# CaiLiLab/MuRaL

Hardware: AMD Instinct MI355X
Metric: predicted bases/s (SNV local=10/distal=1000, 4-class, predict) (higher is better)
Workload: dtype f32; 1 GPU; SNV default predict, synthetic 10M positions (BASELINE.json configs[1]); local_radius=10, distal_radius=1000, n_class=4, input=2-bit packed genome resident in HBM, every site's full window, weights=weights_init, torch.manual_seed(0), parallelism=dp1, collective=none

## Files before the change

### mural_amd/csrc/snv.h

```cpp
#pragma once
#include "common.h"

namespace mural {

constexpr int SNV_C = 32;
constexpr int SNV_K = 3;
constexpr int SNV_NLAYER = 10;
constexpr int SNV_KSTEPS = 24;
constexpr int SNV_WFRAG = 2 * SNV_KSTEPS * 64;
constexpr int SNV_LUT = 125 * SNV_C;
constexpr int SNV_TAPS = 3 * N_SYM * SNV_C;
constexpr int SNV_LUTBLK = SNV_LUT + SNV_TAPS + SNV_C;
constexpr int SNV_LUT4 = 256 * SNV_C;
constexpr int SNV_MAXCLASS = 16;
constexpr int SNV_CHUNK = 131072;
constexpr int SNV_NB2MAX = 9;
constexpr int SNV_THREADS = 256;
constexpr int SNV_WAVES = SNV_THREADS / 64;
constexpr int SNV_MID_HALF = 100;

enum { L_RB1A_C1 = 0, L_RB1A_C2, L_RB1B_C1, L_RB1B_C2, L_CONV2, L_RB2A_C1, L_RB2A_C2, L_RB2B_C1, L_RB2B_C2, L_CONV3 };
enum { EX_RB1_ENTRY = 0, EX_BN_MID = 1, EX_BN_OUT = 2, EX_FC_BN = 3, EX_COUNT = 4 };

struct TowerGeom {
  int L1;
  int col0;
  int L[3];
  int pk[3], ps[3], pp[3];
  int Sc[3];
  int NC[3];
  int nb[3];
  FastDiv dL[3];
  FastDiv dSc[3];
};

struct TowerDev {
  const float* lut;
  const float* lut4;
  const float* taps;
  const float* bias0;
  const float* wfrag;
  const float* wfrag4;
  const float* bias;
  const float* post_s;
  const float* post_t;
  const float* ex_s;
  const float* ex_t;
  const float* fc_w;
  const float* fc_b;
};

struct LocalDev {
  const float* emb;
  const float* w1t;
  const float* b1;
  const float* w2t;
  const float* b2;
  const float* w3t;
  const float* b3;
  const float* frag;
  int frag_floats;
  int cols, emb_rows, in1, h1, h2, n_class;
};

struct LocalMfmaDims { int K1p, K2p, K3p, n1b, n2b, s1, sx, dbg; };

struct Stage1Tower { int L1, col0, L2, pk, ps, pp; };

struct Stage1Args {
  Stage1Tower tw[2];
  const float* lut[2];
  const float* lut4;
  int Lwin, cw, wave_bytes, x0_cols, nwords, radius;
  int64_t n;
  const uint8_t* codes;
  MuralGenome genome;
  const int64_t* pos;
  const uint8_t* strand;
  float* x0;
  const float* dense;
  int32_t* status;
  int loc_on;
  LocalDev loc;
  LocalMfmaDims loc_d;
  const int64_t* loc_cat;
  float* loc_out;
  int* zero;
  int site_mode;
  int dbg_alias;
};

constexpr int FIRST_TRAIN_MAXGRID = 256;
struct FirstFold {
  const float* dz;
  const float* x;
  const float* add1;
  const float* add2;
  const float* state;
  const float* gamma;
  const double* acc;
  double n;
  float* dgamma;
  float* dbeta;
};
struct FirstTrainArgs {
  Stage1Tower tw;
  int Lwin, cw, wave_bytes;
  int64_t B;
  const uint8_t* sym;
  const float* lutblk;
  float* y;
  uint8_t* arg;
  const float* dy;
  float* dpart;
  int cl;
  double* stat;
  FirstFold fold;
  int dbg;
  unsigned long long* stamps;
};
extern unsigned long long* g_first_stamps;
int first_train_grid(int64_t B);
bool first_train_supported(int C, int pk);
int launch_first_train(FirstTrainArgs a, bool bwd, hipStream_t stream);

struct SnvFwdArgs {
  TowerGeom geom[2];
  TowerDev tw[2];
  int P;
  int nbuf;
  int Lwin;
  int n_class;
  int has_local;
  int64_t n;
  const float* x0;
  int x0_cols;
  const float* local_logits;
  float* out;
  float* taps;
  int tap_stride;
  unsigned long long* stamps;
  const int32_t* status;
  int tw_first, tw_last;
  float* xlogit;
  int par;
  float* xlogit2;
  int* tile_count;
  int phase;
  float* s3[2];
  int wave;
  int* unit_counter;
  int seg_n, seg_step, seg_col0;
};

constexpr int RU_EC = 9;
constexpr int RU_EV = 5;
constexpr int RU_L = 2 * RU_EC;
constexpr int RU_SC = RU_L + 1;

struct EdgeArgs {
  TowerDev tw;
  int64_t n;
  const int64_t* pos;
  const uint8_t* strand;
  int64_t glen;
  int64_t t0[2], nb;
  int woff;
  int L1;
  int L2, L3;
  int D;
  int pk2, ps2, pp2;
  int u_lo, u_hi;
  int right_pad;
  const float* F[2];
  const float* El[2];
  const float* Er[2];
  const float* R[2];
  const float* S[2];
  float* s3;
};

constexpr int EW_P = 7;
size_t edge_wave_lds_bytes();
int launch_snv_edge_wave(const EdgeArgs& e, int* unit_counter, hipStream_t stream);

}

struct MuralSnvModel {
  MuralSnvShape shape;
  mural::SnvFwdArgs args;
  mural::SnvFwdArgs args_split[4];
  size_t lds_split[4];
  bool split;
  mural::SnvFwdArgs args_small;
  size_t lds_small;
  mural::LocalDev local;
  float* blob;
  size_t blob_floats;
  size_t lds_bytes;
  mural::Stage1Args s1;
  size_t s1_lds_bytes;
  bool s1_pair;
  bool loc_fused;
  mural::LocalMfmaDims loc_d;
  size_t loc_lds;
  bool longwin;
  bool front_only;
  bool front_mid;
  int lw_nA, lw_LA, lw_LB, lw_SB, lw_nj;
  mural::SnvFwdArgs args_lwA, args_lwB;
  size_t lds_lwA, lds_lwB;
  int64_t chunk;
};

namespace mural {
bool stage1_small_batch(int64_t n);
int launch_snv_stage1(const Stage1Args& a, bool packed, size_t lds_bytes, hipStream_t stream);
int launch_snv_local(const LocalDev& L, const int64_t* cat, int64_t n, float* out, hipStream_t stream);
int launch_snv_towers(const MuralSnvModel* m, const SnvFwdArgs& a, size_t lds_bytes, hipStream_t stream);
int profile_begin();
int profile_end(double* total_ms, int64_t* launches);
size_t plan_wave_geometry(SnvFwdArgs& a, int Lwin, int Pw, int n_class, int tower, int phase);
int launch_snv_tower_wave(const SnvFwdArgs& a, size_t lds_bytes, hipStream_t stream);
int launch_snv_tower_wave_jobs(const SnvFwdArgs* jobs, const size_t* lds_bytes, int n, hipStream_t stream);
extern unsigned long long* g_tower_stamps;
}
```

### mural_amd/csrc/snv_stage1.hip

```cpp
#include <algorithm>
#include <cstdlib>

#include "dense_symbol.h"
#include "snv.h"
#include "snv_local_mfma.h"

namespace mural {

using f32x4 = __attribute__((ext_vector_type(4))) float;
__device__ __forceinline__ f32x4 s1_ld4(const float* p) { return *reinterpret_cast<const f32x4*>(p); }
__device__ __forceinline__ f32x4 s1_max4(f32x4 a, f32x4 b) {
  return f32x4{fmaxf(a.x, b.x), fmaxf(a.y, b.y), fmaxf(a.z, b.z), fmaxf(a.w, b.w)};
}

constexpr int S1_WAVES = 16;
constexpr int S1_THREADS = 64 * S1_WAVES;

__device__ __forceinline__ void wave_lds_fence() { asm volatile("s_waitcnt lgkmcnt(0)" ::: "memory"); }

__device__ __forceinline__ uint32_t kmer_index(const uint8_t* cb, int j, int L1) {
  if (j <= 0 || j >= L1 - 1) return 255u;
  const uint32_t l = cb[j], c = cb[j + 1], r = cb[j + 2];
  return (l <= 4u && c <= 4u && r <= 4u) ? (25u * l + 5u * c + r) : 255u;
}

template <int SLOT>
__device__ __forceinline__ void build_kwin(const Stage1Tower& g, int lane, const uint8_t* cb0, uint8_t* kw, int nl = 64) {
  const uint8_t* cb = cb0 + g.col0;
  const int ndw = g.L2 * (SLOT / 4);
  for (int t = lane; t < ndw; t += nl) {
    const int j2 = t / (SLOT / 4);
    const int w0 = 4 * (t % (SLOT / 4));
    uint32_t packed = 0;
#pragma unroll
    for (int q = 0; q < 4; ++q) {
      const int w = w0 + q;
      const uint32_t idx = (w < g.pk) ? kmer_index(cb, j2 * g.ps - g.pp + w, g.L1) : 255u;
      packed |= idx << (8 * q);
    }
    *reinterpret_cast<uint32_t*>(kw + (size_t)t * 4) = packed;
  }
}

template <int SLOT>
__device__ __forceinline__ void pooled_lookup(const Stage1Tower& g, int lane, const float* lutS, const uint8_t* cb0,
                                              const uint8_t* kw, float* __restrict__ out , int nl = 64) {
  const float* tapS = lutS + SNV_LUT;
  const float* b0S = tapS + SNV_TAPS;
  const uint8_t* cb = cb0 + g.col0;
  const int cg = lane & 7;
  const int total = g.L2 * 8;
  for (int task = lane; task < total; task += nl) {
    const int jt = task >> 3;
    const int j2 = jt == 0 ? g.L2 - 1 : jt - 1;
    uint32_t d[SLOT / 4];
    if (SLOT == 16) {
      const uint4 q = *reinterpret_cast<const uint4*>(kw + (size_t)j2 * 16);
      d[0] = q.x; d[1] = q.y; d[2] = q.z; d[SLOT / 4 - 1] = q.w;
    } else {
      d[0] = *reinterpret_cast<const uint32_t*>(kw + (size_t)j2 * 4);
    }
    uint32_t hi = d[SLOT / 4 - 1] & 0x00FFFFFFu;
#pragma unroll
    for (int r = 0; r + 1 < SLOT / 4; ++r) hi |= d[r];
    const bool fast = ((hi & 0x80808080u) == 0u) && (g.pk == SLOT - 1);
    f32x4 m = f32x4{-INFINITY, -INFINITY, -INFINITY, -INFINITY};
    if (fast) {
#pragma unroll
      for (int w = 0; w < SLOT - 1; ++w) {
        const uint32_t idx = (d[w >> 2] >> (8 * (w & 3))) & 0xFFu;
        m = s1_max4(m, s1_ld4(lutS + idx * 32u + 4u * cg));
      }
    } else {
      const int jlo = j2 * g.ps - g.pp;
      for (int w = 0; w < g.pk; ++w) {
        const int j = jlo + w;
        if (j < 0 || j >= g.L1) continue;
        const uint32_t idx = kmer_index(cb, j, g.L1);
        f32x4 v;
        if (idx != 255u) {
          v = s1_ld4(lutS + idx * 32u + 4u * cg);
        } else {
          const uint32_t sl = (j == 0) ? (uint32_t)SYM_PAD : cb[j];
          const uint32_t sc = cb[j + 1];
          const uint32_t sr = (j == g.L1 - 1) ? (uint32_t)SYM_PAD : cb[j + 2];
          v = s1_ld4(b0S + 4 * cg);
          v += s1_ld4(tapS + (0 * N_SYM + sl) * 32 + 4 * cg);
          v += s1_ld4(tapS + (1 * N_SYM + sc) * 32 + 4 * cg);
          v += s1_ld4(tapS + (2 * N_SYM + sr) * 32 + 4 * cg);
        }
        m = s1_max4(m, v);
      }
    }
    *reinterpret_cast<f32x4*>(out + (size_t)j2 * 32 + 4 * cg) = m;
  }
}

__device__ __forceinline__ void build_kpair(const Stage1Tower& g, int lane, const uint8_t* cb0, uint8_t* kw) {
  const uint8_t* cb = cb0 + g.col0;
  for (int t = lane; t < 2 * g.L2; t += 64) {
    const int j2 = t >> 1, half = t & 1;
    const int j0 = j2 * g.ps - g.pp + 8 * half;
    const int ncol = half ? 7 : 8;
    uint32_t sy[10];
    uint32_t bad = (j0 < 1 || j0 + ncol - 1 > g.L1 - 2) ? 1u : 0u;
#pragma unroll
    for (int i = 0; i < 10; ++i) {
      const int idx = j0 + i;
      const bool in = idx >= 0 && idx <= g.L1 + 1 && i < ncol + 2;
      sy[i] = in ? cb[idx] : 0u;
      if (i < ncol + 2 && (!in || sy[i] > 3u)) bad = 1u;
    }
    uint32_t lo = 0;
#pragma unroll
    for (int q = 0; q < 4; ++q) {
      uint32_t code;
      if (half && q == 3) code = 25u * sy[6] + 5u * sy[7] + sy[8];
      else code = 64u * sy[2 * q] + 16u * sy[2 * q + 1] + 4u * sy[2 * q + 2] + sy[2 * q + 3];
      lo |= (code & 0xFFu) << (8 * q);
    }
    uint32_t* dst = reinterpret_cast<uint32_t*>(kw + (size_t)j2 * 16 + 8 * half);
    dst[0] = lo;
    dst[1] = bad;
  }
}

__device__ __forceinline__ void pooled_lookup_pair(const Stage1Tower& g, int lane, const float* lutS, const float* lut4S, const uint8_t* cb0,
                                                   const uint8_t* kw, float* __restrict__ out ) {
  const float* tapS = lutS + SNV_LUT;
  const float* b0S = tapS + SNV_TAPS;
  const uint8_t* cb = cb0 + g.col0;
  const int cg = lane & 7;
  const int total = g.L2 * 8;
  for (int task = lane; task < total; task += 64) {
    const int jt = task >> 3;
    const int j2 = jt == 0 ? g.L2 - 1 : jt - 1;
    const uint4 q = *reinterpret_cast<const uint4*>(kw + (size_t)j2 * 16);
    f32x4 m;
    if (((q.y | q.w) & 0xFFu) == 0u) {
      m = s1_ld4(lut4S + (q.x & 0xFFu) * 32u + 4u * cg);
      m = s1_max4(m, s1_ld4(lut4S + ((q.x >> 8) & 0xFFu) * 32u + 4u * cg));
      m = s1_max4(m, s1_ld4(lut4S + ((q.x >> 16) & 0xFFu) * 32u + 4u * cg));
      m = s1_max4(m, s1_ld4(lut4S + (q.x >> 24) * 32u + 4u * cg));
      m = s1_max4(m, s1_ld4(lut4S + (q.z & 0xFFu) * 32u + 4u * cg));
      m = s1_max4(m, s1_ld4(lut4S + ((q.z >> 8) & 0xFFu) * 32u + 4u * cg));
      m = s1_max4(m, s1_ld4(lut4S + ((q.z >> 16) & 0xFFu) * 32u + 4u * cg));
      m = s1_max4(m, s1_ld4(lutS + (q.z >> 24) * 32u + 4u * cg));
    } else {
      m = f32x4{-INFINITY, -INFINITY, -INFINITY, -INFINITY};
      const int jlo = j2 * g.ps - g.pp;
      for (int w = 0; w < g.pk; ++w) {
        const int j = jlo + w;
        if (j < 0 || j >= g.L1) continue;
        const uint32_t idx = kmer_index(cb, j, g.L1);
        f32x4 v;
        if (idx != 255u) {
          v = s1_ld4(lutS + idx * 32u + 4u * cg);
        } else {
          const uint32_t sl = (j == 0) ? (uint32_t)SYM_PAD : cb[j];
          const uint32_t sc = cb[j + 1];
          const uint32_t sr = (j == g.L1 - 1) ? (uint32_t)SYM_PAD : cb[j + 2];
          v = s1_ld4(b0S + 4 * cg);
          v += s1_ld4(tapS + (0 * N_SYM + sl) * 32 + 4 * cg);
          v += s1_ld4(tapS + (1 * N_SYM + sc) * 32 + 4 * cg);
          v += s1_ld4(tapS + (2 * N_SYM + sr) * 32 + 4 * cg);
        }
        m = s1_max4(m, v);
      }
    }
    *reinterpret_cast<f32x4*>(out + (size_t)j2 * 32 + 4 * cg) = m;
  }
}

template <int SRC>
__global__ __launch_bounds__(S1_THREADS) void snv_stage1_kernel(const Stage1Args args) {
  extern __shared__ __attribute__((aligned(16))) float s1mem[];
  const int tid = threadIdx.x;
  const int lane = tid & 63;
  const int wave = __builtin_amdgcn_readfirstlane(tid >> 6);
  float* lutL = s1mem;
  float* lutM = s1mem + SNV_LUTBLK;
  const bool pair = args.lut4 != nullptr;
  float* lut4 = s1mem + 2 * SNV_LUTBLK;
  uint8_t* wbase = reinterpret_cast<uint8_t*>(s1mem + 2 * SNV_LUTBLK + (pair ? SNV_LUT4 : 0)) + (size_t)wave * args.wave_bytes;
  uint8_t* cb = wbase;
  uint8_t* kwL = cb + args.cw;
  uint8_t* kwM = kwL + args.tw[0].L2 * 16;

  for (int i = tid * 4; i < SNV_LUTBLK; i += S1_THREADS * 4) {
    *reinterpret_cast<f32x4*>(lutL + i) = s1_ld4(args.lut[0] + i);
    *reinterpret_cast<f32x4*>(lutM + i) = s1_ld4(args.lut[1] + i);
  }
  if (pair)
    for (int i = tid * 4; i < SNV_LUT4; i += S1_THREADS * 4) *reinterpret_cast<f32x4*>(lut4 + i) = s1_ld4(args.lut4 + i);
  __syncthreads();

  const int Lwin = args.Lwin;
  const int64_t stride = (int64_t)gridDim.x * S1_WAVES;
  int64_t row = (int64_t)blockIdx.x * S1_WAVES + wave;
  int64_t pos_pre = 0;
  uint32_t neg_pre = 0;
  if (SRC == 1 && row < args.n) {
    pos_pre = args.pos[row];
    neg_pre = args.strand[row];
  }
  for (; row < args.n; row += stride) {
    if (SRC == 1) {
      const int64_t ws = pos_pre - args.radius;
      const bool neg = neg_pre != 0;
      const int64_t glen = args.genome.length;
      if (row + stride < args.n) {
        pos_pre = args.pos[row + stride];
        neg_pre = args.strand[row + stride];
      }
      if (lane == 0) {
        cb[0] = SYM_PAD;
        cb[Lwin + 1] = SYM_PAD;
      }
      for (int wi = lane; wi < args.nwords; wi += 64) {
        const int64_t w = (ws >> 4) + wi;
        uint32_t word = 0, mword = 0;
        if (w >= 0 && 16 * w < glen) {
          word = args.genome.packed2[w];
          mword = (args.genome.nmask[w >> 1] >> (16u * (uint32_t)(w & 1))) & 0xFFFFu;
        }
        const int j0 = (int)(16 * w - ws);
        if (w < 0 || 16 * w >= glen) mword = 0xFFFFu;
        else if (16 * w + 15 >= glen) mword |= 0xFFFFu << (uint32_t)(glen - 16 * w);
        const uint32_t cw = neg ? ~word : word;
        const int jb = neg ? Lwin - 1 - j0 - 15 : j0;
        uint8_t* dst = cb + jb + 1;
        const bool nfree = (mword & 0xFFFFu) == 0u;
#pragma unroll
        for (int k = 0; k < 16; ++k) {
          const int o = neg ? 15 - k : k;
          uint32_t sym = (cw >> (2 * k)) & 3u;
          if (!nfree) sym = ((mword >> k) & 1u) ? (uint32_t)SYM_N : sym;
          if ((unsigned)(jb + o) < (unsigned)Lwin) dst[o] = (uint8_t)sym;
        }
      }
      if (args.genome.n_amb > 0) {
        const int64_t e0 = amb_lower_bound_wave(args.genome.amb_pos, args.genome.n_amb, ws, lane);
        for (int64_t e = e0 + lane; e < args.genome.n_amb; e += 64) {
          const int64_t gpos = args.genome.amb_pos[e];
          if (gpos >= ws + Lwin) break;
          uint32_t sym = args.genome.amb_sym[e];
          if (neg) sym = sym_complement(sym);
          cb[(int)(neg ? (ws + Lwin - 1 - gpos) : (gpos - ws)) + 1] = (uint8_t)sym;
        }
      }
    } else {
      const uint8_t* src = args.codes + row * Lwin;
      for (int jj = lane; jj < Lwin + 2; jj += 64) {
        const int j = jj - 1;
        cb[jj] = (j >= 0 && j < Lwin) ? src[j] : (uint8_t)SYM_PAD;
      }
    }
    wave_lds_fence();
    if (pair) build_kpair(args.tw[0], lane, cb, kwL);
    else build_kwin<16>(args.tw[0], lane, cb, kwL);
    build_kwin<4>(args.tw[1], lane, cb, kwM);
    wave_lds_fence();
    float* out = args.x0 + (size_t)(args.dbg_alias ? (row & 63) : row) * args.x0_cols * 32;
    if (pair) pooled_lookup_pair(args.tw[0], lane, lutL, lut4, cb, kwL, out);
    else pooled_lookup<16>(args.tw[0], lane, lutL, cb, kwL, out);
    pooled_lookup<4>(args.tw[1], lane, lutM, cb, kwM, out + (size_t)args.tw[0].L2 * 32);
    wave_lds_fence();
  }
}

template <int SRC>
__global__ __launch_bounds__(S1_THREADS) void snv_stage1_site_kernel(const Stage1Args args) {
  extern __shared__ __attribute__((aligned(16))) float s1mem[];
  const int tid = threadIdx.x;
  if (args.loc_on && (int64_t)blockIdx.x == args.n) {
    if (tid < LOC_THREADS) local_mlp_mfma_body(args.loc, args.loc_cat, args.n, args.loc_out, args.loc_d, s1mem, 0, 1);
    return;
  }
  float* lutL = s1mem;
  float* lutM = s1mem + SNV_LUTBLK;
  uint8_t* cb = reinterpret_cast<uint8_t*>(s1mem + 2 * SNV_LUTBLK);
  uint8_t* kwL = cb + args.cw;
  uint8_t* kwM = kwL + args.tw[0].L2 * 16;
  for (int i = tid * 4; i < SNV_LUTBLK; i += S1_THREADS * 4) {
    *reinterpret_cast<f32x4*>(lutL + i) = s1_ld4(args.lut[0] + i);
    *reinterpret_cast<f32x4*>(lutM + i) = s1_ld4(args.lut[1] + i);
  }
  const int Lwin = args.Lwin;
  if (args.zero != nullptr && blockIdx.x == 0)
    for (int64_t i = tid; i < args.n; i += S1_THREADS) args.zero[i] = 0;
  for (int64_t row = blockIdx.x; row < args.n; row += gridDim.x) {
    __syncthreads();
    if (SRC == 1) {
      const int64_t ws = args.pos[row] - args.radius;
      const bool neg = args.strand[row] != 0;
      if (tid == 0) {
        cb[0] = SYM_PAD;
        cb[Lwin + 1] = SYM_PAD;
      }
      for (int j = tid; j < Lwin; j += S1_THREADS) {
        const int64_t gpos = neg ? ws + Lwin - 1 - j : ws + j;
        uint32_t sym = genome_sym_iupac(args.genome, gpos);
        if (neg) sym = sym_complement(sym);
        cb[j + 1] = (uint8_t)sym;
      }
    } else if (SRC == 2) {
      const float* src = args.dense + (size_t)row * 4 * Lwin;
      if (tid == 0) {
        cb[0] = SYM_PAD;
        cb[Lwin + 1] = SYM_PAD;
      }
      bool bad = false;
      for (int j0 = tid; j0 < Lwin; j0 += 2 * S1_THREADS) {
        const int j1 = j0 + S1_THREADS;
        const int j1c = j1 < Lwin ? j1 : j0;
        float v[2][4];
#pragma unroll
        for (int ch = 0; ch < 4; ++ch) {
          v[0][ch] = src[(size_t)ch * Lwin + j0];
          v[1][ch] = src[(size_t)ch * Lwin + j1c];
        }
        int s0 = dense_symbol(v[0][0], v[0][1], v[0][2], v[0][3]);
        int s1 = dense_symbol(v[1][0], v[1][1], v[1][2], v[1][3]);
        bad |= (s0 < 0) | (s1 < 0);
        cb[j0 + 1] = (uint8_t)(s0 < 0 ? SYM_N : s0);
        if (j1 < Lwin) cb[j1 + 1] = (uint8_t)(s1 < 0 ? SYM_N : s1);
      }
      if (bad && args.status != nullptr) atomicOr(args.status, (int)MURAL_E_ENCODING);
    } else {
      const uint8_t* src = args.codes + row * Lwin;
      for (int jj = tid; jj < Lwin + 2; jj += S1_THREADS) {
        const int j = jj - 1;
        cb[jj] = (j >= 0 && j < Lwin) ? src[j] : (uint8_t)SYM_PAD;
      }
    }
    __syncthreads();
    build_kwin<16>(args.tw[0], tid, cb, kwL, S1_THREADS);
    build_kwin<4>(args.tw[1], tid, cb, kwM, S1_THREADS);
    __syncthreads();
    float* out = args.x0 + (size_t)row * args.x0_cols * 32;
    pooled_lookup<16>(args.tw[0], tid, lutL, cb, kwL, out, S1_THREADS);
    pooled_lookup<4>(args.tw[1], tid, lutM, cb, kwM, out + (size_t)args.tw[0].L2 * 32, S1_THREADS);
  }
}


template <int SLOT>
__device__ __forceinline__ void pooled_lookup_train(const Stage1Tower& g, int lane, const float* lutS, const uint8_t* cb0,
                                                    const uint8_t* kw, float* __restrict__ y ,
                                                    uint8_t* __restrict__ arg , int cl, f32x4& sum1, f32x4& sum2) {
  const float* tapS = lutS + SNV_LUT;
  const float* b0S = tapS + SNV_TAPS;
  const uint8_t* cb = cb0 + g.col0;
  const int cg = lane & 7;
  const int total = g.L2 * 8;
  for (int task = lane; task < total; task += 64) {
    const int j2 = task >> 3;
    uint32_t d[SLOT / 4];
    if (SLOT == 16) {
      const uint4 q = *reinterpret_cast<const uint4*>(kw + (size_t)j2 * 16);
      d[0] = q.x; d[1] = q.y; d[2] = q.z; d[SLOT / 4 - 1] = q.w;
    } else {
      d[0] = *reinterpret_cast<const uint32_t*>(kw + (size_t)j2 * 4);
    }
    uint32_t hi = d[SLOT / 4 - 1] & 0x00FFFFFFu;
#pragma unroll
    for (int r = 0; r + 1 < SLOT / 4; ++r) hi |= d[r];
    const bool fast = ((hi & 0x80808080u) == 0u) && (g.pk == SLOT - 1);
    float m[4] = {-INFINITY, -INFINITY, -INFINITY, -INFINITY};
    uint32_t am[4] = {0u, 0u, 0u, 0u};
    if (fast) {
#pragma unroll
      for (int w = 0; w < SLOT - 1; ++w) {
        const uint32_t idx = (d[w >> 2] >> (8 * (w & 3))) & 0xFFu;
        const f32x4 v = s1_ld4(lutS + idx * 32u + 4u * cg);
#pragma unroll
        for (int q = 0; q < 4; ++q) {
          const bool gt = v[q] > m[q];
          m[q] = gt ? v[q] : m[q];
          am[q] = gt ? (uint32_t)w : am[q];
        }
      }
    } else {
      const int jlo = j2 * g.ps - g.pp;
      for (int w = 0; w < g.pk; ++w) {
        const int j = jlo + w;
        if (j < 0 || j >= g.L1) continue;
        const uint32_t idx = kmer_index(cb, j, g.L1);
        f32x4 v;
        if (idx != 255u) {
          v = s1_ld4(lutS + idx * 32u + 4u * cg);
        } else {
          const uint32_t sl = (j == 0) ? (uint32_t)SYM_PAD : cb[j];
          const uint32_t sc = cb[j + 1];
          const uint32_t sr = (j == g.L1 - 1) ? (uint32_t)SYM_PAD : cb[j + 2];
          v = s1_ld4(b0S + 4 * cg);
          v += s1_ld4(tapS + (0 * N_SYM + sl) * 32 + 4 * cg);
          v += s1_ld4(tapS + (1 * N_SYM + sc) * 32 + 4 * cg);
          v += s1_ld4(tapS + (2 * N_SYM + sr) * 32 + 4 * cg);
        }
#pragma unroll
        for (int q = 0; q < 4; ++q) {
          const bool gt = v[q] > m[q];
          m[q] = gt ? v[q] : m[q];
          am[q] = gt ? (uint32_t)w : am[q];
        }
      }
    }
    if (cl) {
      *reinterpret_cast<f32x4*>(y + (size_t)j2 * 32 + 4 * cg) = f32x4{m[0], m[1], m[2], m[3]};
      const f32x4 r = f32x4{fmaxf(m[0], 0.f), fmaxf(m[1], 0.f), fmaxf(m[2], 0.f), fmaxf(m[3], 0.f)};
      sum1 += r;
      sum2 += f32x4{r.x * r.x, r.y * r.y, r.z * r.z, r.w * r.w};
    } else {
#pragma unroll
      for (int q = 0; q < 4; ++q) y[(size_t)(4 * cg + q) * g.L2 + j2] = m[q];
    }
    *reinterpret_cast<uint32_t*>(arg + (size_t)j2 * 32 + 4 * cg) = am[0] | (am[1] << 8) | (am[2] << 16) | (am[3] << 24);
  }
}

template <int SLOT>
__device__ __forceinline__ void pooled_scatter(const Stage1Tower& g, int lane, float* acc, const uint8_t* cb0,
                                               const uint8_t* kw, const float* __restrict__ dy ,
                                               const uint8_t* __restrict__ arg , int cl) {
  float* tapA = acc + SNV_LUT;
  float* b0A = tapA + SNV_TAPS;
  const uint8_t* cb = cb0 + g.col0;
  const int cg = lane & 7;
  const int total = g.L2 * 8;
  float bsum[4] = {0.f, 0.f, 0.f, 0.f};
  constexpr int NT = 6;
  for (int t0 = lane; t0 < total; t0 += 64 * NT) {
    uint32_t awv[NT];
    f32x4 gv[NT];
#pragma unroll
    for (int u = 0; u < NT; ++u) {
      const int task = t0 + 64 * u;
      const int j2 = (task < total ? task : t0) >> 3;
      awv[u] = *reinterpret_cast<const uint32_t*>(arg + (size_t)j2 * 32 + 4 * cg);
      if (cl) {
        gv[u] = *reinterpret_cast<const f32x4*>(dy + (size_t)j2 * 32 + 4 * cg);
      } else {
#pragma unroll
        for (int q = 0; q < 4; ++q) gv[u][q] = dy[(size_t)(4 * cg + q) * g.L2 + j2];
      }
    }
#pragma unroll
    for (int u = 0; u < NT; ++u) {
      const int task = t0 + 64 * u;
      if (task >= total) break;
      const int j2 = task >> 3;
      const uint32_t aw = awv[u];
      const int jlo = j2 * g.ps - g.pp;
#pragma unroll
      for (int q = 0; q < 4; ++q) {
        const int c = 4 * cg + q;
        const float gq = gv[u][q];
        const int w = (int)((aw >> (8 * q)) & 0xFFu);
        const uint32_t idx = kw[(size_t)j2 * SLOT + w];
        bsum[q] += gq;
        if (idx != 255u) {
          atomicAdd(&acc[idx * 32u + c], gq);
        } else {
          const int j = jlo + w;
          const uint32_t sl = (j == 0) ? (uint32_t)SYM_PAD : cb[j];
          const uint32_t sc = cb[j + 1];
          const uint32_t sr = (j == g.L1 - 1) ? (uint32_t)SYM_PAD : cb[j + 2];
          atomicAdd(&tapA[(0 * N_SYM + sl) * 32 + c], gq);
          atomicAdd(&tapA[(1 * N_SYM + sc) * 32 + c], gq);
          atomicAdd(&tapA[(2 * N_SYM + sr) * 32 + c], gq);
        }
      }
    }
  }
#pragma unroll
  for (int q = 0; q < 4; ++q) {
    float v = bsum[q];
    v += __shfl_xor(v, 8);
    v += __shfl_xor(v, 16);
    v += __shfl_xor(v, 32);
    if (lane < 8) atomicAdd(&b0A[4 * cg + q], v);
  }
}

#define FT_STAMP(K) do { if (a.stamps && tid == 0) a.stamps[8 * blockIdx.x + (K)] = __builtin_amdgcn_s_memrealtime(); } while (0)


template <int SLOT>
__device__ __forceinline__ void pooled_scatter_cl(const Stage1Tower& g, int lane, float* acc, const uint8_t* cb0, const uint8_t* kw,
                                                  const float* __restrict__ dy , const uint8_t* __restrict__ arg ,
                                                  int dbg) {
  float* tapA = acc + SNV_LUT;
  float* b0A = tapA + SNV_TAPS;
  const uint8_t* cb = cb0 + g.col0;
  const int c = lane & 31, h = lane >> 5;
  const int npair = (g.L2 + 1) >> 1;
  float bsum = 0.f;
  const __amdgpu_buffer_rsrc_t gd = __builtin_amdgcn_make_buffer_rsrc(const_cast<float*>(dy), 0, (dbg & 2) ? 0 : g.L2 * 128, 0x00020000);
  const __amdgpu_buffer_rsrc_t ad = __builtin_amdgcn_make_buffer_rsrc(const_cast<uint8_t*>(arg), 0, (dbg & 2) ? 0 : g.L2 * 32, 0x00020000);
  constexpr int NT = 16;
  for (int p0 = 0; p0 < npair; p0 += NT) {
    float gv[NT];
    uint32_t awv[NT];
    const uint32_t go = 4u * (uint32_t)lane + 256u * (uint32_t)p0, ao = (uint32_t)lane + 64u * (uint32_t)p0;
    int hh = h;
    asm volatile("" : "+v"(hh));
#pragma unroll
    for (int u = 0; u < NT; ++u) {
      awv[u] = __builtin_amdgcn_raw_buffer_load_b8(ad, ao + 64u * u, 0, 0);
      gv[u] = __builtin_bit_cast(float, __builtin_amdgcn_raw_buffer_load_b32(gd, go + 256u * u, 0, 0));
    }
#pragma unroll
    for (int u = 0; u < NT; ++u) {
      const int j2 = 2 * (p0 + u) + hh;
      if (j2 < g.L2) {
        const float gq = gv[u];
        const int w = (int)(awv[u] & 0xFFu);
        const uint32_t idx = (dbg & 4) ? (uint32_t)(j2 & 63) : kw[j2 * SLOT + w];
        bsum += gq;
        if (dbg & 1) continue;
        const int j = j2 * g.ps - g.pp + w;
        const uint32_t sl = (j == 0) ? (uint32_t)SYM_PAD : cb[j];
        const bool tab = idx != 255u;
        atomicAdd(tab ? &acc[idx * 32u + c] : &tapA[(0 * N_SYM + sl) * 32 + c], gq);
        if (!tab) {
          const uint32_t sc = cb[j + 1];
          const uint32_t sr = (j == g.L1 - 1) ? (uint32_t)SYM_PAD : cb[j + 2];
          atomicAdd(&tapA[(1 * N_SYM + sc) * 32 + c], gq);
          atomicAdd(&tapA[(2 * N_SYM + sr) * 32 + c], gq);
        }
      }
      if ((u & 3) == 3) __builtin_amdgcn_sched_barrier(0);
    }
  }
  bsum += __shfl_xor(bsum, 32);
  if (lane < 32) atomicAdd(&b0A[c], bsum);
}

template <int SLOT, bool BWD>
__global__ __launch_bounds__(S1_THREADS) void first_train_kernel(const FirstTrainArgs a) {
  extern __shared__ __attribute__((aligned(16))) float s1mem[];
  const int tid = threadIdx.x;
  FT_STAMP(0);
  const int lane = tid & 63;
  const int wave = __builtin_amdgcn_readfirstlane(tid >> 6);
  float* blk = s1mem;
  uint8_t* cb = reinterpret_cast<uint8_t*>(s1mem + SNV_LUTBLK) + (size_t)wave * a.wave_bytes;
  uint8_t* kw = cb + a.cw;
  for (int i = tid * 4; i < SNV_LUTBLK; i += S1_THREADS * 4)
    *reinterpret_cast<f32x4*>(blk + i) = BWD ? f32x4{0.f, 0.f, 0.f, 0.f} : s1_ld4(a.lutblk + i);
  __syncthreads();
  FT_STAMP(1);
  const Stage1Tower g = a.tw;
  const int Lwin = a.Lwin;
  f32x4 sum1 = f32x4{0.f, 0.f, 0.f, 0.f}, sum2 = f32x4{0.f, 0.f, 0.f, 0.f};
  for (int64_t row = (int64_t)blockIdx.x * S1_WAVES + wave; row < a.B; row += (int64_t)gridDim.x * S1_WAVES) {
    const uint8_t* src = a.sym + row * Lwin;
    constexpr int UN = 8;
    for (int jj0 = lane; jj0 < Lwin + 2; jj0 += 64 * UN) {
      uint8_t v[UN];
#pragma unroll
      for (int u = 0; u < UN; ++u) {
        const int j = jj0 + 64 * u - 1;
        v[u] = (j >= 0 && j < Lwin) ? src[j] : (uint8_t)SYM_PAD;
      }
#pragma unroll
      for (int u = 0; u < UN; ++u)
        if (jj0 + 64 * u < Lwin + 2) cb[jj0 + 64 * u] = v[u];
    }
    wave_lds_fence();
    FT_STAMP(2);
    build_kwin<SLOT>(g, lane, cb, kw);
    wave_lds_fence();
    FT_STAMP(3);
    const size_t o = (size_t)row * 32 * g.L2;
    if (BWD) pooled_scatter<SLOT>(g, lane, blk, cb, kw, a.dy + o, a.arg + o, a.cl);
    else pooled_lookup_train<SLOT>(g, lane, blk, cb, kw, a.y + o, a.arg + o, a.cl, sum1, sum2);
    wave_lds_fence();
    FT_STAMP(4);
  }
  if (!BWD && a.stat) {
    __syncthreads();
    float* red = blk;
#pragma unroll
    for (int q = 0; q < 4; ++q) {
      float v1 = sum1[q], v2 = sum2[q];
#pragma unroll
      for (int off = 8; off < 64; off <<= 1) {
        v1 += __shfl_xor(v1, off);
        v2 += __shfl_xor(v2, off);
      }
      if (lane < 8) {
        red[wave * 64 + 4 * lane + q] = v1;
        red[wave * 64 + 32 + 4 * lane + q] = v2;
      }
    }
    __syncthreads();
    if (tid < 64) {
      float v = 0.f;
#pragma unroll
      for (int w = 0; w < S1_WAVES; ++w) v += red[w * 64 + tid];
      atomicAdd(&a.stat[(size_t)(blockIdx.x % MURAL_BN_SLOTS) * 64 + tid], (double)v);
    }
  }
  if (BWD) {
    __syncthreads();
    FT_STAMP(5);
    float* dst = a.dpart + (size_t)blockIdx.x * SNV_LUTBLK;
    for (int i = tid * 4; i < SNV_LUTBLK; i += S1_THREADS * 4) *reinterpret_cast<f32x4*>(dst + i) = s1_ld4(blk + i);
  }
  FT_STAMP(6);
}


constexpr int FB_ROWS = 13;
template <bool FOLD>
__global__ __launch_bounds__(S1_THREADS) void first_bwd_cl_kernel(const FirstTrainArgs a) {
  extern __shared__ __attribute__((aligned(16))) float s1mem[];
  const int tid = threadIdx.x;
  const int lane = tid & 63;
  const int wave = __builtin_amdgcn_readfirstlane(tid >> 6);
  FT_STAMP(0);
  float* rare = s1mem;
  float* red = rare + SNV_TAPS;
  uint8_t* cb0 = reinterpret_cast<uint8_t*>(red + S1_WAVES * FB_ROWS * 32) + (size_t)wave * a.cw;
  for (int i = tid; i < SNV_TAPS; i += S1_THREADS) rare[i] = 0.f;
  const int c = lane & 31, h = lane >> 5;
  float k0 = 0.f, m1 = 0.f, m2 = 0.f, mu = 0.f, is = 0.f;
  if constexpr (FOLD) {
    float* fc = red;
    if (tid < 32) {
      double s1 = 0.0, s2 = 0.0;
      for (int k = 0; k < MURAL_BN_SLOTS; ++k) {
        s1 += a.fold.acc[((size_t)k * 2 + 0) * 32 + tid];
        s2 += a.fold.acc[((size_t)k * 2 + 1) * 32 + tid];
      }
      fc[tid] = a.fold.gamma[tid] * a.fold.state[3 * 32 + tid];
      fc[32 + tid] = (float)(s1 / a.fold.n);
      fc[64 + tid] = (float)(s2 / a.fold.n);
      fc[96 + tid] = a.fold.state[2 * 32 + tid];
      fc[128 + tid] = a.fold.state[3 * 32 + tid];
      if (blockIdx.x == 0) {
        a.fold.dgamma[tid] = (float)s2;
        a.fold.dbeta[tid] = (float)s1;
      }
    }
    __syncthreads();
    k0 = fc[c]; m1 = fc[32 + c]; m2 = fc[64 + c]; mu = fc[96 + c]; is = fc[128 + c];
  }
  __syncthreads();
  FT_STAMP(1);
  const Stage1Tower g = a.tw;
  const int Lwin = a.Lwin;
  const int npair = (g.L2 + 1) >> 1;
  const uint8_t* cb = cb0 + g.col0;
  float acc[3][4];
#pragma unroll
  for (int t = 0; t < 3; ++t)
#pragma unroll
    for (int q = 0; q < 4; ++q) acc[t][q] = 0.f;
  float bsum = 0.f;
  for (int64_t row = (int64_t)blockIdx.x * S1_WAVES + wave; row < a.B; row += (int64_t)gridDim.x * S1_WAVES) {
    const uint8_t* src = a.sym + row * Lwin;
    constexpr int UN = 8;
    for (int jj0 = lane; jj0 < Lwin + 2; jj0 += 64 * UN) {
      uint8_t v[UN];
#pragma unroll
      for (int u = 0; u < UN; ++u) {
        const int j = jj0 + 64 * u - 1;
        v[u] = (j >= 0 && j < Lwin) ? src[j] : (uint8_t)SYM_PAD;
      }
#pragma unroll
      for (int u = 0; u < UN; ++u)
        if (jj0 + 64 * u < Lwin + 2) cb0[jj0 + 64 * u] = v[u];
    }
    wave_lds_fence();
    FT_STAMP(2);
    const size_t o = (size_t)row * 32 * g.L2;
    const int gbytes = g.L2 * 128;
    const __amdgpu_buffer_rsrc_t gd = __builtin_amdgcn_make_buffer_rsrc(const_cast<float*>((FOLD ? a.fold.dz : a.dy) + o), 0, gbytes, 0x00020000);
    const __amdgpu_buffer_rsrc_t ad = __builtin_amdgcn_make_buffer_rsrc(a.arg + o, 0, g.L2 * 32, 0x00020000);
    auto opt = [&](const float* p) __attribute__((always_inline)) {
      return __builtin_amdgcn_make_buffer_rsrc(const_cast<float*>(p ? p + o : a.dy), 0, p ? gbytes : 0, 0x00020000);
    };
    const __amdgpu_buffer_rsrc_t xd = opt(FOLD ? a.fold.x : nullptr), r1d = opt(FOLD ? a.fold.add1 : nullptr), r2d = opt(FOLD ? a.fold.add2 : nullptr);
    constexpr int NT = FOLD ? 8 : 16;
    for (int p0 = 0; p0 < npair; p0 += NT) {
      float gv[NT];
      uint32_t awv[NT];
      const uint32_t go = 4u * (uint32_t)lane + 256u * (uint32_t)p0, ao = (uint32_t)lane + 64u * (uint32_t)p0;
      int hh = h;
      asm volatile("" : "+v"(hh));
      if constexpr (FOLD) {
        float xv[NT], r1[NT], r2[NT];
#pragma unroll
        for (int u = 0; u < NT; ++u) {
          awv[u] = __builtin_amdgcn_raw_buffer_load_b8(ad, ao + 64u * u, 0, 0);
          gv[u] = __builtin_bit_cast(float, __builtin_amdgcn_raw_buffer_load_b32(gd, go + 256u * u, 0, 0));
          xv[u] = __builtin_bit_cast(float, __builtin_amdgcn_raw_buffer_load_b32(xd, go + 256u * u, 0, 0));
          r1[u] = __builtin_bit_cast(float, __builtin_amdgcn_raw_buffer_load_b32(r1d, go + 256u * u, 0, 0));
          r2[u] = __builtin_bit_cast(float, __builtin_amdgcn_raw_buffer_load_b32(r2d, go + 256u * u, 0, 0));
        }
#pragma unroll
        for (int u = 0; u < NT; ++u) {
          const float xh = (xv[u] - mu) * is;
          const float gq = k0 * ((gv[u] - m1) - xh * m2);
          gv[u] = ((xv[u] > 0.f ? gq : 0.f) + r1[u]) + r2[u];
        }
      } else {
#pragma unroll
        for (int u = 0; u < NT; ++u) {
          awv[u] = __builtin_amdgcn_raw_buffer_load_b8(ad, ao + 64u * u, 0, 0);
          gv[u] = __builtin_bit_cast(float, __builtin_amdgcn_raw_buffer_load_b32(gd, go + 256u * u, 0, 0));
        }
      }
#pragma unroll
      for (int u = 0; u < NT; ++u) {
        const int j2 = 2 * (p0 + u) + hh;
        const float gq = j2 < g.L2 ? gv[u] : 0.f;
        const int j = (j2 < g.L2 ? j2 : g.L2 - 1) * g.ps - g.pp + (int)(awv[u] & 0xFFu);
        uint32_t sy[3] = {cb[j], cb[j + 1], cb[j + 2]};
        sy[0] = j == 0 ? (uint32_t)SYM_PAD : sy[0];
        sy[2] = j == g.L1 - 1 ? (uint32_t)SYM_PAD : sy[2];
        bsum += gq;
#pragma unroll
        for (int t = 0; t < 3; ++t)
#pragma unroll
          for (int q = 0; q < 4; ++q) acc[t][q] += sy[t] == (uint32_t)q ? gq : 0.f;
        if ((sy[0] | sy[1] | sy[2]) > 3u) {
#pragma unroll
          for (int t = 0; t < 3; ++t)
            if (sy[t] > 3u) atomicAdd(&rare[(t * N_SYM + sy[t]) * 32 + c], gq);
        }
        if ((u & 3) == 3) __builtin_amdgcn_sched_barrier(0);
      }
    }
    wave_lds_fence();
    FT_STAMP(4);
  }
#pragma unroll
  for (int t = 0; t < 3; ++t)
#pragma unroll
    for (int q = 0; q < 4; ++q) {
      const float v = acc[t][q] + __shfl_xor(acc[t][q], 32);
      if (lane < 32) red[(wave * FB_ROWS + 4 * t + q) * 32 + c] = v;
    }
  {
    const float v = bsum + __shfl_xor(bsum, 32);
    if (lane < 32) red[(wave * FB_ROWS + 12) * 32 + c] = v;
  }
  __syncthreads();
  FT_STAMP(5);
  float* dst = a.dpart + (size_t)blockIdx.x * SNV_LUTBLK;
  for (int i = tid * 4; i < SNV_LUT; i += S1_THREADS * 4) *reinterpret_cast<f32x4*>(dst + i) = f32x4{0.f, 0.f, 0.f, 0.f};
  for (int i = tid; i < SNV_TAPS + 32; i += S1_THREADS) {
    const int t = i / (N_SYM * 32), r = i - t * N_SYM * 32, sym = r >> 5, cc = r & 31;
    const int k = i >= SNV_TAPS ? 12 : (sym < 4 ? 4 * t + sym : -1);
    float v = i < SNV_TAPS ? rare[i] : 0.f;
    if (k >= 0) {
      const int ch = i >= SNV_TAPS ? i - SNV_TAPS : cc;
#pragma unroll
      for (int w = 0; w < S1_WAVES; ++w) v += red[(w * FB_ROWS + k) * 32 + ch];
    }
    dst[SNV_LUT + i] = v;
  }
  FT_STAMP(6);
}

#undef FT_STAMP

unsigned long long* g_first_stamps = nullptr;

int first_train_grid(int64_t B) {
  const int64_t want = (B + S1_WAVES - 1) / S1_WAVES;
  return (int)(want < 1 ? 1 : (want < FIRST_TRAIN_MAXGRID ? want : FIRST_TRAIN_MAXGRID));
}

bool first_train_supported(int C, int pk) { return C == SNV_C && pk >= 1 && pk <= 15; }

int launch_first_train(FirstTrainArgs a, bool bwd, hipStream_t stream) {
  if (a.B == 0) return MURAL_OK;
  MURAL_REQUIRE(first_train_supported(SNV_C, a.tw.pk), "first layer: pool window %d not supported by the table kernel", a.tw.pk);
  const int slot = a.tw.pk <= 3 ? 4 : 16;
  a.cw = (a.Lwin + 2 + 15) & ~15;
  a.wave_bytes = a.cw + ((a.tw.L2 * slot + 15) & ~15);
  const size_t lds = (size_t)SNV_LUTBLK * 4 + (size_t)S1_WAVES * a.wave_bytes;
  MURAL_REQUIRE(lds <= 160 * 1024, "first layer: window of %d columns does not fit the LDS working set", a.Lwin);
  using KernelFn = void (*)(const FirstTrainArgs);
  MURAL_REQUIRE(!a.fold.dz || (bwd && a.cl), "first layer: the folded BatchNorm-backward apply belongs to the channel-last backward");
  if (bwd && a.cl && (a.fold.dz || !dev_env("MURAL_DEBUG_FIRST_SCATTER"))) {
    const size_t lds_b = (size_t)(SNV_TAPS + S1_WAVES * FB_ROWS * 32) * 4 + (size_t)S1_WAVES * a.cw;
    MURAL_REQUIRE(lds_b <= 160 * 1024, "first layer: window of %d columns does not fit the LDS working set", a.Lwin);
    static DynLdsOnce big_b;
    if (int rc = big_b.ensure(&first_bwd_cl_kernel<false>, &first_bwd_cl_kernel<true>)) return rc;
    a.stamps = g_first_stamps;
    if (a.fold.dz) hipLaunchKernelGGL(first_bwd_cl_kernel<true>, dim3(first_train_grid(a.B)), dim3(S1_THREADS), lds_b, stream, a);
    else hipLaunchKernelGGL(first_bwd_cl_kernel<false>, dim3(first_train_grid(a.B)), dim3(S1_THREADS), lds_b, stream, a);
    MURAL_HIP_CHECK(hipGetLastError());
    return MURAL_OK;
  }
  KernelFn fn = slot == 4 ? (bwd ? first_train_kernel<4, true> : first_train_kernel<4, false>)
                          : (bwd ? first_train_kernel<16, true> : first_train_kernel<16, false>);
  static DynLdsOnce big_lds[4];
  if (int rc = big_lds[(slot == 4 ? 0 : 2) + (bwd ? 1 : 0)].ensure(fn)) return rc;
  a.stamps = g_first_stamps;
  static const int dbg = dev_int("MURAL_DEBUG_FIRST", 0);
  a.dbg = dbg;
  hipLaunchKernelGGL(fn, dim3(first_train_grid(a.B)), dim3(S1_THREADS), lds, stream, a);
  MURAL_HIP_CHECK(hipGetLastError());
  return MURAL_OK;
}

bool stage1_small_batch(int64_t n) { return n <= 256 && !dev_env("MURAL_DEBUG_NO_SMALL_BATCH"); }

int launch_snv_stage1(const Stage1Args& a, bool packed, size_t lds_bytes, hipStream_t stream) {
  if (a.n == 0) return MURAL_OK;
  MURAL_REQUIRE(a.dense == nullptr || (!packed && stage1_small_batch(a.n)), "stage 1: the dense source is the small-batch kernel's");
  MURAL_REQUIRE(!a.loc_on || stage1_small_batch(a.n), "stage 1: the local-branch workgroup is the small-batch kernel's");
  static DynLdsOnce big_lds;
  if (int rc = big_lds.ensure(&snv_stage1_kernel<0>, &snv_stage1_kernel<1>, &snv_stage1_site_kernel<0>, &snv_stage1_site_kernel<1>,
                              &snv_stage1_site_kernel<2>))
    return rc;
  if (stage1_small_batch(a.n) || a.site_mode) {
    const unsigned grid = stage1_small_batch(a.n) ? (unsigned)a.n + (a.loc_on ? 1u : 0u) : (unsigned)std::min<int64_t>(a.n, 16384);
    if (!packed && a.dense != nullptr)
      hipLaunchKernelGGL(snv_stage1_site_kernel<2>, dim3(grid), dim3(S1_THREADS), lds_bytes, stream, a);
    else if (packed) hipLaunchKernelGGL(snv_stage1_site_kernel<1>, dim3(grid), dim3(S1_THREADS), lds_bytes, stream, a);
    else hipLaunchKernelGGL(snv_stage1_site_kernel<0>, dim3(grid), dim3(S1_THREADS), lds_bytes, stream, a);
    MURAL_HIP_CHECK(hipGetLastError());
    return MURAL_OK;
  }
  const int64_t want = (a.n + S1_WAVES - 1) / S1_WAVES;
  const int grid = (int)(want < 256 ? want : 256);
  Stage1Args b = a;
  static const int alias = dev_env("MURAL_DEBUG_S1_ALIAS") ? 1 : 0;
  b.dbg_alias = alias;
  if (packed)
    hipLaunchKernelGGL(snv_stage1_kernel<1>, dim3(grid), dim3(S1_THREADS), lds_bytes, stream, b);
  else
    hipLaunchKernelGGL(snv_stage1_kernel<0>, dim3(grid), dim3(S1_THREADS), lds_bytes, stream, b);
  MURAL_HIP_CHECK(hipGetLastError());
  return MURAL_OK;
}

}
```

Before: 17.20 million bases/s.

## Build k-mer indices directly from packed 2-bit words for N-free windows

Adds a fast path in the packed stage-1 kernel. When a window has no N or out-of-genome bases (checked with a wave ballot over the mask words), the raw 2-bit words go into LDS, reversed or complemented per strand. The k-mer pair and trinucleotide indices are then computed with alignbit and bit arithmetic, skipping the per-base symbol unpacking, and only the edge symbols that pooled lookup still reads are written out. Kernel arguments are read through the kernarg segment pointer to cut register pressure. This relies on a narrow geometry check and on unused LDS space inside the symbol buffer, so any mismatch could silently corrupt results.

```diff
diff --git a/mural_amd/csrc/snv.h b/mural_amd/csrc/snv.h
--- a/mural_amd/csrc/snv.h
+++ b/mural_amd/csrc/snv.h
@@ -87,6 +87,7 @@
   float* loc_out;
   int* zero;
   int site_mode;
+  int clean_ok;
   int dbg_alias;
 };
 
diff --git a/mural_amd/csrc/snv_stage1.hip b/mural_amd/csrc/snv_stage1.hip
--- a/mural_amd/csrc/snv_stage1.hip
+++ b/mural_amd/csrc/snv_stage1.hip
@@ -172,6 +172,65 @@
   }
 }
 
+constexpr int S1_WOFF = 32;
+
+__device__ __forceinline__ uint32_t s1_rev2(uint32_t w) {
+  const uint32_t r = __builtin_bitreverse32(w);
+  return ((r >> 1) & 0x55555555u) | ((r & 0x55555555u) << 1);
+}
+__device__ __forceinline__ uint32_t s1_base5(uint32_t x6) { return x6 + 9u * (x6 >> 4) + ((x6 >> 2) & 3u); }
+__device__ __forceinline__ uint32_t s1_fields(const uint32_t* wsm, int t, int tmax) {
+  t = t < 0 ? 0 : (t > tmax ? tmax : t);
+  return __builtin_amdgcn_alignbit(wsm[(t >> 4) + 1], wsm[t >> 4], 2u * ((uint32_t)t & 15u));
+}
+
+__device__ __forceinline__ void build_kpair_bits(int L1, int L2, int lane, const uint32_t* wsm, int T0, int tmax, uint8_t* kw) {
+  for (int t = lane; t < 2 * L2; t += 64) {
+    const int j2 = t >> 1, half = t & 1;
+    const int j0 = j2 * 15 - 7 + 8 * half;
+    const int ncol = half ? 7 : 8;
+    const uint32_t bad = (j0 < 1 || j0 + ncol - 1 > L1 - 2) ? 1u : 0u;
+    const uint32_t x = s1_fields(wsm, T0 - (j0 + 8), tmax);
+    const uint32_t last = half ? s1_base5((x >> 2) & 63u) : (x & 0xFFu);
+    const uint32_t lo = ((x >> 12) & 0xFFu) | (((x >> 8) & 0xFFu) << 8) | (((x >> 4) & 0xFFu) << 16) | (last << 24);
+    *reinterpret_cast<uint2*>(kw + (size_t)j2 * 16 + 8 * half) = uint2{lo, bad};
+  }
+}
+
+__device__ __forceinline__ void build_kwin3_bits(int L1, int L2, int lane, const uint32_t* wsm, int T0, int tmax, uint8_t* kw) {
+  for (int j2 = lane; j2 < L2; j2 += 64) {
+    const int j = 3 * j2 - 1;
+    const uint32_t x = s1_fields(wsm, T0 - (j + 3), tmax);
+    const uint32_t i0 = (j > 0 && j < L1 - 1) ? s1_base5((x >> 4) & 63u) : 255u;
+    const uint32_t i1 = (j + 1 > 0 && j + 1 < L1 - 1) ? s1_base5((x >> 2) & 63u) : 255u;
+    const uint32_t i2 = (j + 2 > 0 && j + 2 < L1 - 1) ? s1_base5(x & 63u) : 255u;
+    *reinterpret_cast<uint32_t*>(kw + (size_t)j2 * 4) = i0 | (i1 << 8) | (i2 << 16) | 0xFF000000u;
+  }
+}
+
+__device__ __forceinline__ void clean_edge_symbols(const Stage1Tower& gl, const Stage1Tower& gm, int Lwin, int lane, const uint32_t* wsm,
+                                                   int T0, uint8_t* cb) {
+  int c;
+  if (lane < 16) c = lane;
+  else if (lane < 40) c = 15 * (gl.L2 - 1) - 8 + (lane - 16);
+  else if (lane < 48) c = gm.col0 - 1 + (lane - 40);
+  else c = gm.col0 + 3 * (gm.L2 - 1) - 2 + (lane - 48);
+  if (c >= 0 && c < Lwin) {
+    const int t = T0 - c;
+    cb[c + 1] = (uint8_t)((wsm[t >> 4] >> (2u * ((uint32_t)t & 15u))) & 3u);
+  }
+}
+
+using S1Kernarg = const __attribute__((address_space(4))) Stage1Args;
+__device__ __forceinline__ S1Kernarg* s1_kernarg() {
+  S1Kernarg* p = (S1Kernarg*)__builtin_amdgcn_kernarg_segment_ptr();
+  asm volatile("" : "+s"(p));
+  return p;
+}
+__device__ __forceinline__ Stage1Tower s1_tower(S1Kernarg* ka, int i) {
+  return Stage1Tower{ka->tw[i].L1, ka->tw[i].col0, ka->tw[i].L2, ka->tw[i].pk, ka->tw[i].ps, ka->tw[i].pp};
+}
+
 template <int SRC>
 __global__ __launch_bounds__(S1_THREADS) void snv_stage1_kernel(const Stage1Args args) {
   extern __shared__ __attribute__((aligned(16))) float s1mem[];
@@ -196,6 +255,7 @@
   __syncthreads();
 
   const int Lwin = args.Lwin;
+  const int64_t n = args.n;
   const int64_t stride = (int64_t)gridDim.x * S1_WAVES;
   int64_t row = (int64_t)blockIdx.x * S1_WAVES + wave;
   int64_t pos_pre = 0;
@@ -204,25 +264,66 @@
     pos_pre = args.pos[row];
     neg_pre = args.strand[row];
   }
-  for (; row < args.n; row += stride) {
+  for (; row < n; row += stride) {
+    S1Kernarg* ka = s1_kernarg();
+    bool clean = false;
+    int T0 = 0;
     if (SRC == 1) {
-      const int64_t ws = pos_pre - args.radius;
+      const int64_t ws = pos_pre - ka->radius;
       const bool neg = neg_pre != 0;
-      const int64_t glen = args.genome.length;
-      if (row + stride < args.n) {
-        pos_pre = args.pos[row + stride];
-        neg_pre = args.strand[row + stride];
+      const int64_t glen = ka->genome.length;
+      if (row + stride < ka->n) {
+        pos_pre = ka->pos[row + stride];
+        neg_pre = ka->strand[row + stride];
       }
       if (lane == 0) {
         cb[0] = SYM_PAD;
         cb[Lwin + 1] = SYM_PAD;
       }
-      for (int wi = lane; wi < args.nwords; wi += 64) {
+      clean = false;
+      if (ka->clean_ok) {
+        const int nw = ka->nwords;
+        const int off = (int)(ws & 15);
+        uint32_t wd[2], dirty = 0;
+#pragma unroll
+        for (int r = 0; r < 2; ++r) {
+          const int wi = lane + 64 * r;
+          const int64_t w = (ws >> 4) + wi;
+          uint32_t word = 0, mword = 0xFFFFu;
+          if (wi < nw && w >= 0 && 16 * w < glen) {
+            word = ka->genome.packed2[w];
+            mword = (ka->genome.nmask[w >> 1] >> (16u * (uint32_t)(w & 1))) & 0xFFFFu;
+            if (16 * w + 15 >= glen) mword |= 0xFFFFu << (uint32_t)(glen - 16 * w);
+          }
+          const int j0 = 16 * wi - off;
+          const int blo = j0 < 0 ? -j0 : 0;
+          const int bhi = Lwin - j0 < 0 ? 0 : (Lwin - j0 > 16 ? 16 : Lwin - j0);
+          const uint32_t inwin = wi < nw ? (((1u << bhi) - 1u) & (0xFFFFFFFFu << blo)) : 0u;
+          dirty |= mword & inwin;
+          wd[r] = word;
+        }
+        clean = __builtin_amdgcn_ballot_w64(dirty != 0u) == 0ull;
+        if (clean) {
+          uint32_t* wsm = reinterpret_cast<uint32_t*>(cb + S1_WOFF);
+#pragma unroll
+          for (int r = 0; r < 2; ++r) {
+            const int wi = lane + 64 * r;
+            if (wi < nw) wsm[neg ? 1 + wi : nw - wi] = neg ? ~wd[r] : s1_rev2(wd[r]);
+          }
+          if (lane == 0) {
+            wsm[0] = 0u;
+            wsm[nw + 1] = 0u;
+          }
+          T0 = 16 + (neg ? off + Lwin - 1 : 16 * nw - 1 - off);
+        }
+      }
+      if (!clean) {
+      for (int wi = lane; wi < ka->nwords; wi += 64) {
         const int64_t w = (ws >> 4) + wi;
         uint32_t word = 0, mword = 0;
         if (w >= 0 && 16 * w < glen) {
-          word = args.genome.packed2[w];
-          mword = (args.genome.nmask[w >> 1] >> (16u * (uint32_t)(w & 1))) & 0xFFFFu;
+          word = ka->genome.packed2[w];
+          mword = (ka->genome.nmask[w >> 1] >> (16u * (uint32_t)(w & 1))) & 0xFFFFu;
         }
         const int j0 = (int)(16 * w - ws);
         if (w < 0 || 16 * w >= glen) mword = 0xFFFFu;
@@ -239,32 +340,49 @@
           if ((unsigned)(jb + o) < (unsigned)Lwin) dst[o] = (uint8_t)sym;
         }
       }
-      if (args.genome.n_amb > 0) {
-        const int64_t e0 = amb_lower_bound_wave(args.genome.amb_pos, args.genome.n_amb, ws, lane);
-        for (int64_t e = e0 + lane; e < args.genome.n_amb; e += 64) {
-          const int64_t gpos = args.genome.amb_pos[e];
+      if (ka->genome.n_amb > 0) {
+        const int64_t e0 = amb_lower_bound_wave(ka->genome.amb_pos, ka->genome.n_amb, ws, lane);
+        for (int64_t e = e0 + lane; e < ka->genome.n_amb; e += 64) {
+          const int64_t gpos = ka->genome.amb_pos[e];
           if (gpos >= ws + Lwin) break;
-          uint32_t sym = args.genome.amb_sym[e];
+          uint32_t sym = ka->genome.amb_sym[e];
           if (neg) sym = sym_complement(sym);
           cb[(int)(neg ? (ws + Lwin - 1 - gpos) : (gpos - ws)) + 1] = (uint8_t)sym;
         }
       }
+      }
     } else {
-      const uint8_t* src = args.codes + row * Lwin;
+      const uint8_t* src = ka->codes + row * Lwin;
       for (int jj = lane; jj < Lwin + 2; jj += 64) {
         const int j = jj - 1;
         cb[jj] = (j >= 0 && j < Lwin) ? src[j] : (uint8_t)SYM_PAD;
       }
     }
     wave_lds_fence();
-    if (pair) build_kpair(args.tw[0], lane, cb, kwL);
-    else build_kwin<16>(args.tw[0], lane, cb, kwL);
-    build_kwin<4>(args.tw[1], lane, cb, kwM);
+    ka = s1_kernarg();
+    {
+      const Stage1Tower gl = s1_tower(ka, 0), gm = s1_tower(ka, 1);
+      if (SRC == 1 && clean) {
+        const uint32_t* wsm = reinterpret_cast<const uint32_t*>(cb + S1_WOFF);
+        const int tmax = 16 * ka->nwords + 15;
+        build_kpair_bits(gl.L1, gl.L2, lane, wsm, T0, tmax, kwL);
+        build_kwin3_bits(gm.L1, gm.L2, lane, wsm, T0 - gm.col0, tmax, kwM);
+        clean_edge_symbols(gl, gm, Lwin, lane, wsm, T0, cb);
+      } else {
+        if (pair) build_kpair(gl, lane, cb, kwL);
+        else build_kwin<16>(gl, lane, cb, kwL);
+        build_kwin<4>(gm, lane, cb, kwM);
+      }
+    }
     wave_lds_fence();
-    float* out = args.x0 + (size_t)(args.dbg_alias ? (row & 63) : row) * args.x0_cols * 32;
-    if (pair) pooled_lookup_pair(args.tw[0], lane, lutL, lut4, cb, kwL, out);
-    else pooled_lookup<16>(args.tw[0], lane, lutL, cb, kwL, out);
-    pooled_lookup<4>(args.tw[1], lane, lutM, cb, kwM, out + (size_t)args.tw[0].L2 * 32);
+    ka = s1_kernarg();
+    {
+      const Stage1Tower gl = s1_tower(ka, 0), gm = s1_tower(ka, 1);
+      float* out = ka->x0 + (size_t)(ka->dbg_alias ? (row & 63) : row) * ka->x0_cols * 32;
+      if (pair) pooled_lookup_pair(gl, lane, lutL, lut4, cb, kwL, out);
+      else pooled_lookup<16>(gl, lane, lutL, cb, kwL, out);
+      pooled_lookup<4>(gm, lane, lutM, cb, kwM, out + (size_t)gl.L2 * 32);
+    }
     wave_lds_fence();
   }
 }
@@ -836,6 +954,10 @@
   Stage1Args b = a;
   static const int alias = dev_env("MURAL_DEBUG_S1_ALIAS") ? 1 : 0;
   b.dbg_alias = alias;
+  const Stage1Tower &gl = a.tw[0], &gm = a.tw[1];
+  b.clean_ok = packed && a.lut4 != nullptr && gl.pk == 15 && gl.ps == 15 && gl.pp == 7 && gl.col0 == 0 && gl.L1 == a.Lwin && gm.pk == 3 &&
+               gm.ps == 3 && gm.pp == 1 && gm.col0 + gm.L1 <= a.Lwin && a.nwords <= 128 && S1_WOFF + 4 * (a.nwords + 2) <= gm.col0 &&
+               a.genome.n_amb == 0;
   if (packed)
     hipLaunchKernelGGL(snv_stage1_kernel<1>, dim3(grid), dim3(S1_THREADS), lds_bytes, stream, b);
   else
```

After: 17.29 million bases/s (median of 6 runs). About the same (+0.5%).
